# JINXER000/GIE-mapping

Hardware: AMD Instinct MI355X
Metric: edt_map_update_throughput (higher is better)
Workload: dtype int32; 1 GPU; 512x512x512 @ 0.05 m, sensor-less hash world (BASELINE config 5): occupied iff hash(x,y,z) < 1 %, full observation, 25 ~; preset=c5, fast_mode=False, tiles=single volume, blocks=360448

## Files before the change

gie-mapping_amd/csrc/gie_functors.h:

```cpp
#ifndef GIE_FUNCTORS_H
#define GIE_FUNCTORS_H

#include "gie_ops.h"


struct op_classify_depth {
    GIE_DEVM bool tile_skip(const gie_ctx &, int, int, int) const { return false; } const float *img; gie_cam_param p;
    GIE_DEVM bool skip(const gie_ctx &, int, int, int, int) const { return false; }
    GIE_DEVM void operator()(const gie_ctx &c, int x, int y, int z) const {
        const int t = gie_classify_depth(c, img, p, x, y, z);
        if (t != GIE_VOX_UNKNOWN) { c.inst_type[gie_lid(c, x, y, z)] = (int8_t)t; gie_mark_block_needed(c, x, y, z); } } };
struct op_classify_multiscan {
    const float *img; gie_multiscan_param p; float tan_lo, tan_hi; int fov_test;
    GIE_DEVM bool tile_skip(const gie_ctx &c, int x, int y, int z0) const {
        if (!fov_test || c.for_motion_planner || !(tan_hi >= 0.f && tan_lo <= 0.f)) return false;
        const float w = c.voxel_width;
        const int z1 = (z0 + 7 < c.Z) ? z0 + 7 : c.Z - 1;
        float ax, ay, az, bx, by, bz;
        gie_se3_apply(c.G2L, (float)(x + c.pvt[0]) * w, (float)(y + c.pvt[1]) * w, (float)(z0 + c.pvt[2]) * w, &ax, &ay, &az);
        gie_se3_apply(c.G2L, (float)(x + c.pvt[0]) * w, (float)(y + c.pvt[1]) * w, (float)(z1 + c.pvt[2]) * w, &bx, &by, &bz);
        const float ha = sqrtf(ay * ay + ax * ax), hb = sqrtf(by * by + bx * bx);
        return (az > ha * tan_hi && bz > hb * tan_hi) || (az < ha * tan_lo && bz < hb * tan_lo);
    }
    GIE_DEVM bool skip(const gie_ctx &c, int, int x, int y, int z) const {
// ... 40 lines not shown
    GIE_DEVM void load1(const gie_ctx &c, int id, int x, int y, int z, st &s) const { gie_mark_load1(c, id, x, y, z, s); }
    GIE_DEVM void load2(const gie_ctx &c, int, int, int, int, st &s) const { gie_mark_load2(c, s); }
    GIE_DEVM int finish(const gie_ctx &c, int id, int x, int y, int z, const st &s) const { gie_mark_finish(c, id, x, y, z, s); return 0; }
    GIE_DEVM void operator()(const gie_ctx &c, int x, int y, int z) const { gie_mark_voxel(c, x, y, z); } };
struct op_markc {
    typedef gie_markc_st st;
    GIE_DEVM bool tile_skip(const gie_ctx &c, int x, int y, int z0) const { return !c.tknown[gie_tile_index(c, x, y, z0)]; }
    GIE_DEVM bool skip(const gie_ctx &c, int id, int, int, int) const { return c.glb_type[id] == GIE_VOX_UNKNOWN; }
    GIE_DEVM void load1(const gie_ctx &c, int id, int x, int y, int z, st &s) const { gie_markc_load1(c, id, x, y, z, s); }
    GIE_DEVM void load2(const gie_ctx &c, int, int, int, int, st &s) const { gie_markc_load2(c, s); }
    GIE_DEVM int finish(const gie_ctx &c, int id, int x, int y, int z, const st &s) const { return gie_markc_finish(c, id, x, y, z, s); }
    GIE_DEVM void column_max(const gie_ctx &c, int x, int y, int z0, unsigned known, unsigned valid, int vmax) const { gie_markc_column(c, x, y, z0, known, valid, vmax); }
    GIE_DEVM int operator()(const gie_ctx &c, int x, int y, int z) const { return gie_markc_voxel(c, x, y, z); } };
struct op_commit {
    typedef gie_commit_st st;
    GIE_DEVM bool tile_skip(const gie_ctx &c, int x, int y, int z0) const { return c.cnt[GIE_CNT_BARFAIL] != 0 || !c.tknown[gie_tile_index(c, x, y, z0)]; }
    GIE_DEVM bool skip(const gie_ctx &c, int id, int, int, int) const { return c.glb_type[id] == GIE_VOX_UNKNOWN; }
    GIE_DEVM void load1(const gie_ctx &c, int id, int x, int y, int z, st &s) const { gie_commit_load1(c, id, x, y, z, s); }
    GIE_DEVM void load2(const gie_ctx &, int, int, int, int, st &) const {}
    GIE_DEVM int finish(const gie_ctx &c, int id, int, int, int, const st &s) const { gie_commit_finish(c, id, s); return 0; }
    GIE_DEVM void operator()(const gie_ctx &c, int x, int y, int z) const { gie_commit_voxel(c, x, y, z); } };

struct op_frontier {
    typedef gie_frontier_st st;
    GIE_DEVM bool tile_skip(const gie_ctx &c, int x, int y, int z0) const { return c.tsum[gie_tile_index(c, x, y, z0)] == 0; }
    GIE_DEVM bool skip(const gie_ctx &c, int id, int x, int y, int z) const {
        if (c.glb_type[id] == GIE_VOX_UNKNOWN) return true;
        const bool on_face = x == 0 || y == 0 || z == 0 || x == c.X - 1 || y == c.Y - 1 || z == c.Z - 1;
        return !on_face && c.tsum[gie_tile_index(c, x, y, z)] == 2;
    }
    GIE_DEVM void load1(const gie_ctx &c, int id, int x, int y, int z, st &s) const { gie_frontier_load1(c, id, x, y, z, s); }
    GIE_DEVM void load2(const gie_ctx &, int, int, int, int, st &) const {}
    GIE_DEVM int finish(const gie_ctx &c, int id, int x, int y, int z, const st &s) const { push_seed(c, gie_frontier_finish(c, id, x, y, z, s), id); return 0; }
    GIE_DEVM void operator()(const gie_ctx &c, int x, int y, int z) const { push_seed(c, gie_frontier_voxel(c, x, y, z), gie_lid(c, x, y, z)); }
    GIE_DEVM void push_seed(const gie_ctx &c, const int push, const int id) const {
        const unsigned long long m = __ballot(push);
        if (m) {
            const int lane = __lane_id();
            const int leader = __ffsll((long long)m) - 1;
            int base = 0;
            if (lane == leader) base = gie_aadd32(&c.cnt[GIE_CNT_C], __popcll(m));
            base = __shfl(base, leader);
            if (push) {
                const int slot = base + __popcll(m & ((1ull << lane) - 1ull));
                if (slot < c.qcap_c) c.qc[0][slot] = id;
                else gie_aor32(&c.cnt[GIE_CNT_ERR], GIE_ERRF_QUEUE);
            }
        }
    }
};

struct op_tile_summary {
    GIE_DEVM static int unk(const gie_ctx &c, int t) { return c.tunk[t] | (c.tact[t] ^ 1); }
    GIE_DEVM static uint8_t value(const gie_ctx &c, int t) {
        if (!c.tknown[t]) return 0;
        const int tx = t % c.tfd[0], ty = (t / c.tfd[0]) % c.tfd[1], tz = t / (c.tfd[0] * c.tfd[1]);
        const bool face = tx == 0 || ty == 0 || tz == 0 || tx == c.tfd[0] - 1 || ty == c.tfd[1] - 1 || tz == c.tfd[2] - 1;
        const int sx = 1, sy = c.tfd[0], sz = c.tfd[0] * c.tfd[1];
        int w = unk(c, t) | c.tflag[t];
        if (tx > 0) w |= unk(c, t - sx) | c.tflag[t - sx];
        if (tx < c.tfd[0] - 1) w |= unk(c, t + sx) | c.tflag[t + sx];
        if (ty > 0) w |= unk(c, t - sy) | c.tflag[t - sy];
        if (ty < c.tfd[1] - 1) w |= unk(c, t + sy) | c.tflag[t + sy];
        if (tz > 0) w |= unk(c, t - sz) | c.tflag[t - sz];
        if (tz < c.tfd[2] - 1) w |= unk(c, t + sz) | c.tflag[t + sz];
        return w ? 1 : (face ? 2 : 0);
    }
    GIE_DEVM void operator()(const gie_ctx &c, int t) const {
        const bool real = t >= 0;
        if (!real) t = 0;
        const uint8_t v = real ? value(c, t) : 0;
        if (real) c.tsum[t] = v;
        const int slot = gie_wg_reserve(&c.cnt[GIE_CNT_TL_FRONT], v == 1);
        if (slot >= 0) c.tl_front[slot] = t | (c.tlazy[t] ? (int32_t)0x80000000 : 0);
    } };
struct op_halo_export { int face; gie_halo_voxel *out; GIE_DEVM void operator()(const gie_ctx &c, int i) const { gie_halo_export_voxel(c, face, i, out); } };
struct op_halo_need { int face; const gie_halo_voxel *in; GIE_DEVM void operator()(const gie_ctx &c, int i) const { gie_halo_need_voxel(c, face, i, in); } };
struct op_halo_import { int face; const gie_halo_voxel *in; GIE_DEVM void operator()(const gie_ctx &c, int i) const { gie_halo_import_voxel(c, face, i, in); } };
struct op_halo_export_sparse { int face; gie_halo_entry *out; int32_t *count; GIE_DEVM void operator()(const gie_ctx &c, int i) const { gie_halo_export_sparse_voxel(c, face, i, out, count); } };
struct op_halo_need_sparse { int face, nface; const gie_halo_entry *in; const int32_t *count; GIE_DEVM void operator()(const gie_ctx &c, int j) const { gie_halo_need_entry(c, face, j, in, count, nface); } };
struct op_halo_import_sparse { int face, nface; const gie_halo_entry *in; const int32_t *count; GIE_DEVM void operator()(const gie_ctx &c, int j) const { gie_halo_import_entry(c, face, j, in, count, nface); } };
struct gie_face_set { int off[7]; GIE_DEVM int face_of(int i) const { int f = 0; while (f < 5 && i >= off[f + 1]) f++; return f; } };
struct op_halo_export_all { gie_face_set fs; gie_halo_voxel *out[6];
    GIE_DEVM void operator()(const gie_ctx &c, int i) const { const int f = fs.face_of(i); gie_halo_export_voxel(c, f, i - fs.off[f], out[f]); } };
struct op_halo_need_all { gie_face_set fs; const gie_halo_voxel *in[6];
    GIE_DEVM void operator()(const gie_ctx &c, int i) const { const int f = fs.face_of(i); gie_halo_need_voxel(c, f, i - fs.off[f], in[f]); } };
struct op_halo_import_all { gie_face_set fs; const gie_halo_voxel *in[6];
    GIE_DEVM void operator()(const gie_ctx &c, int i) const { const int f = fs.face_of(i); gie_halo_import_voxel(c, f, i - fs.off[f], in[f]); } };
struct op_refine { GIE_DEVM void operator()(const gie_ctx &c, int j) const {
        const int id = gie_refine_entry(c, j);
        if (id >= 0 && gie_refine_voxel(c, id)) gie_push32(c, c.qc[0], &c.cnt[GIE_CNT_C], c.qcap_c, id);
    } };
struct op_register_point { const float *xyz; float *g; GIE_DEVM void operator()(const gie_ctx &c, int i) const { gie_register_point(c, xyz, g, i); } };
struct op_query { const int32_t *xyz; gie_voxel *out; GIE_DEVM void operator()(const gie_ctx &c, int i) const { gie_query_voxel(c, xyz, i, out); } };
struct op_fuse_list { GIE_DEVM void operator()(const gie_ctx &c, int t) const {
        const int v = t >= 0 ? gie_fuse_tile_listed(c, t) : 0;
        const int slot = gie_wg_reserve(&c.cnt[GIE_CNT_TL_FUSE], v != 0);
        if (slot >= 0) c.tl_front[slot] = t;
    } };
struct op_pair_flush { gie_flush_boxes b; GIE_DEVM void operator()(const gie_ctx &c, int i) const { gie_pair_flush_voxel(c, b, i); } };
struct op_nbr_check { int32_t *bad; GIE_DEVM void operator()(const gie_ctx &c, int i) const {
        const int slot = i / 6, k = i - 6 * slot;
        if (slot >= c.pool_count[0] || c.g_key[slot] == GIE_KEY_EMPTY) return;
        int b[3];
        gie_unpack_crd(c.g_key[slot], &b[0], &b[1], &b[2]);
        b[k >> 1] += (k & 1) ? 1 : -1;
        const int row = c.g_nbr[8 * (size_t)slot + k];
        const int named = (row >= 0 && row < c.max_blocks && c.g_key[row] == gie_pack_crd(b[0], b[1], b[2])) ? row : -1;
        if (named != gie_hash_find(c, b[0], b[1], b[2])) {
            gie_aadd32(bad, 1);
        }
    } };
struct op_evict { GIE_DEVM void operator()(const gie_ctx &c, int slot) const { if (slot < c.pool_count[0]) gie_evict_slot(c, slot); } };
struct op_rehash { GIE_DEVM void operator()(const gie_ctx &c, int slot) const { if (slot < c.pool_count[0]) gie_rehash_slot(c, slot); } };
struct op_stream_list { const int32_t *rank; int32_t *list; GIE_DEVM void operator()(const gie_ctx &c, int i) const { gie_stream_list(c, rank, list, i); } };
struct op_stream_gather { const int32_t *list; int first; int32_t *keys; gie_voxel *out;
    GIE_DEVM void operator()(const gie_ctx &c, int i) const { gie_stream_gather(c, list, first, keys, out, i); } };
struct op_stream_clear { const int32_t *list; int first; GIE_DEVM void operator()(const gie_ctx &c, int i) const { gie_stream_clear(c, list, first, i); } };
struct op_export_pair { int32_t *d; int32_t *coc; GIE_DEVM void operator()(const gie_ctx &c, int i) const { gie_export_pair(c, i, d, coc); } };
// ... 9 lines not shown
```

gie-mapping_amd/csrc/gie_hip.hip:

```cpp
#include <cstdio>
#include <unistd.h>
#include <cstring>
#include <cstdlib>
#include <string>
#include <algorithm>
#include <vector>
#include <hip/hip_runtime.h>
#include <hip/hip_ext.h>
#include <rocprim/rocprim.hpp>
#include "gie_kernels.hip.h"

#define GIE_NEV 8

struct be_state {
    int device;
    int num_cu;
    int cu_total;
    hipStream_t stream;
    hipEvent_t ev[GIE_NEV];
    int ev_set[GIE_NEV];
    void *scan_tmp; size_t scan_bytes;
    void *arena;
    hipEvent_t copy_ev[2];
    hipStream_t side;
    hipEvent_t side_ready, side_done; int side_on, side_busy;
    int prof_on;
    std::vector<hipEvent_t> *pool;
    std::vector<int> *pending;
    int pool_used;
    int cur_id;
    double acc_ms[32]; int acc_n[32];
};

struct be_arena { char *base; size_t size, top; int k; std::vector<long long> skew; };
static void gie_set_err(const std::string &s);

#define GIE_HIP_OK(expr) do { hipError_t e_ = (expr); if (e_ != hipSuccess) { gie_set_err(std::string(#expr) + ": " + hipGetErrorString(e_)); } } while (0)

#include <mutex>
static std::mutex g_waves_mutex;
static hipEvent_t g_waves_event[64];
static bool g_waves_event_set[64];
static int g_live_mappers[64];

static int be_init(be_state *b, int device, int wave_workgroups)
{
    int n = 0;
    if (hipGetDeviceCount(&n) != hipSuccess || n <= 0) { gie_set_err("no HIP device visible (libgie_hip.so needs an AMD GPU; there is no CPU fallback)"); return 1; }
    if (device < 0 || device >= n) { gie_set_err("bad device_id"); return 1; }
    b->device = device;
    if (hipSetDevice(device) != hipSuccess) { gie_set_err("hipSetDevice failed"); return 1; }
    { hipDeviceProp_t pr; b->num_cu = (hipGetDeviceProperties(&pr, device) == hipSuccess && pr.multiProcessorCount > 0) ? pr.multiProcessorCount : 64; }
    b->cu_total = b->num_cu;
    b->num_cu = b->num_cu >= 64 ? b->num_cu / 2 : b->num_cu;
    if (wave_workgroups > 0) b->num_cu = wave_workgroups < b->cu_total ? wave_workgroups : b->cu_total;
    {
        int per_cu = 0, per_cu_c = 0;
        hipError_t oe = hipOccupancyMaxActiveBlocksPerMultiprocessor(&per_cu, reinterpret_cast<const void *>(&k_waves_ab), GIE_WAVE_THREADS, 0);
        if (oe == hipSuccess) oe = hipOccupancyMaxActiveBlocksPerMultiprocessor(&per_cu_c, reinterpret_cast<const void *>(&k_waves_c), GIE_WAVE_THREADS, 0);
        if (per_cu_c < per_cu) per_cu = per_cu_c;
        if (oe != hipSuccess || per_cu < 1) {
            gie_set_err(std::string("the wavefront kernels cannot be resident on this device (occupancy query: ") + hipGetErrorString(oe) + ", " + std::to_string(per_cu) + " workgroups per compute unit)");
            (void)hipGetLastError();
            return 1;
        }
        if (b->num_cu > per_cu * b->cu_total) b->num_cu = per_cu * b->cu_total;
    }
    if (hipStreamCreateWithFlags(&b->stream, hipStreamNonBlocking) != hipSuccess) { gie_set_err("hipStreamCreate failed"); return 1; }
    for (int i = 0; i < GIE_NEV; i++) { GIE_HIP_OK(hipEventCreate(&b->ev[i])); b->ev_set[i] = 0; }
    b->scan_tmp = nullptr; b->scan_bytes = 0; b->arena = nullptr; b->side_on = 0; b->side_busy = 0;
    for (int i = 0; i < 2; i++) GIE_HIP_OK(hipEventCreateWithFlags(&b->copy_ev[i], hipEventDisableTiming));
    b->prof_on = 0; b->cur_id = -1; b->pool = new std::vector<hipEvent_t>(); b->pending = new std::vector<int>(); b->pool_used = 0;
    for (int i = 0; i < 32; i++) { b->acc_ms[i] = 0; b->acc_n[i] = 0; }
    {
        std::lock_guard<std::mutex> lock(g_waves_mutex);
        if (++g_live_mappers[device & 63] == 2) (void)hipDeviceSynchronize();
    }
    return 0;
}
static void be_fini(be_state *b)
{
    { std::lock_guard<std::mutex> lock(g_waves_mutex); g_live_mappers[b->device & 63]--; }
    if (b->scan_tmp) (void)hipFree(b->scan_tmp);
    for (hipEvent_t e : *b->pool) (void)hipEventDestroy(e);
    delete b->pool; delete b->pending;
    for (int i = 0; i < GIE_NEV; i++) (void)hipEventDestroy(b->ev[i]);
    for (int i = 0; i < 2; i++) (void)hipEventDestroy(b->copy_ev[i]);
    (void)hipStreamDestroy(b->stream);
    if (b->side_on) { (void)hipStreamSynchronize(b->side); (void)hipEventDestroy(b->side_ready); (void)hipEventDestroy(b->side_done); (void)hipStreamDestroy(b->side); }
    if (b->arena) { be_arena *a = (be_arena *)b->arena; if (a->base) (void)hipFree(a->base); delete a; b->arena = nullptr; }
}
static be_arena *be_arena_of(be_state *b)
{
#if !defined(GIE_TEST_HOOKS)
    (void)b; return nullptr;
#else
    static const char *e = getenv("GIE_ARENA_MB");
    if (!e || atoll(e) <= 0) return nullptr;
    if (!b->arena) {
        be_arena *a = new be_arena();
        a->size = (size_t)atoll(e) << 20; a->top = 0; a->k = 0; a->base = nullptr;
        if (const char *sk = getenv("GIE_ARENA_SKEW")) { std::string t(sk); size_t i = 0; while (i < t.size()) { size_t j = t.find(',', i); if (j == std::string::npos) j = t.size(); a->skew.push_back(atoll(t.substr(i, j - i).c_str())); i = j + 1; } }
        if (hipMalloc((void **)&a->base, a->size) != hipSuccess) { a->base = nullptr; a->size = 0; }
        b->arena = a;
    }
    return (be_arena *)b->arena;
#endif
}
static void *be_alloc(be_state *b, size_t bytes, bool zero)
{
    void *p = nullptr;
    (void)hipSetDevice(b->device);
    be_arena *a = bytes >= ((size_t)64 << 20) ? be_arena_of(b) : nullptr;
    if (a && a->base) {
        const size_t sk = (size_t)((a->k < (int)a->skew.size() ? a->skew[a->k] : 0) << 20);
        const size_t at = ((a->top + ((size_t)2 << 20) - 1) & ~(((size_t)2 << 20) - 1)) + sk;
        if (at + bytes <= a->size) { p = a->base + at; a->top = at + bytes; a->k++; }
    }
    if (!p && hipMalloc(&p, bytes ? bytes : 1) != hipSuccess) return nullptr;
    if (zero) GIE_HIP_OK(hipMemsetAsync(p, 0, bytes, b->stream));
    return p;
}
static void be_free(be_state *b, void *p)
{
    (void)hipStreamSynchronize(b->stream);
    be_arena *a = (be_arena *)b->arena;
    if (a && a->base && (char *)p >= a->base && (char *)p < a->base + a->size) return;
    (void)hipFree(p);
}
static void be_memset(be_state *b, void *p, int v, size_t bytes) { GIE_HIP_OK(hipMemsetAsync(p, v, bytes, b->stream)); }
static void be_h2d(be_state *b, void *d, const void *h, size_t bytes)
{
    GIE_HIP_OK(hipMemcpyAsync(d, h, bytes, hipMemcpyHostToDevice, b->stream));
    GIE_HIP_OK(hipStreamSynchronize(b->stream));
}
static void be_d2h(be_state *b, void *h, const void *d, size_t bytes)
// ... 205 lines not shown
}
static int be_edt_z_stream(be_state *b, const gie_ctx &c, int full);
static void be_edt_z_rest(be_state *b, const gie_ctx &c, int full, int zs)
{
    if (zs == 2) gie_launch_edt_dim(b, c, c.X, false, full, 0, true);
    gie_launch_edt_dim(b, c, c.Z, true, full);
}
static void be_edt_z(be_state *b, const gie_ctx &c, int full) { be_edt_z_rest(b, c, full, be_edt_z_stream(b, c, full) ? be_zs_mode(c) : 0); }
#define GIE_VOXA_MULT 32
template <bool STAGED, class F> static void be_vox_list(be_state *b, const gie_ctx &c, const F &f, const int32_t *list, int count_idx, int always_list)
{
    GIE_LAUNCH(b, (k_voxa<F, STAGED>), dim3(b->cu_total * GIE_VOXA_MULT), dim3(256), 0, c, f, list, count_idx, always_list);
}
#define GIE_MARKC_MULT 64
#define GIE_MARKC_LAZY_MULT 40
static void be_markc(be_state *b, const gie_ctx &c, const int32_t *list)
{
    const dim3 g(b->cu_total * ((c.coc_defer && c.lazy_ok) ? GIE_MARKC_LAZY_MULT : GIE_MARKC_MULT)), t(256);
    GIE_LAUNCH(b, k_markc, g, t, 0, c, list);
}
static float be_place_probe(be_state *b, const gie_ctx &c, int reps, int streams = 15)
{
    const long long ntile = (long long)c.tfd[0] * c.tfd[1] * c.tfd[2];
    const int nslot = (int)(ntile < c.max_blocks ? ntile : c.max_blocks);
    hipEvent_t e0, e1;
    if (hipEventCreate(&e0) != hipSuccess || hipEventCreate(&e1) != hipSuccess) return -1.f;
    std::vector<float> ms;
    hipLaunchKernelGGL(k_place_probe, dim3(b->cu_total * GIE_MARKC_MULT), dim3(256), 0, b->stream, c, nslot, streams);
    for (int r = 0; r < reps; r++) {
        (void)hipEventRecord(e0, b->stream);
        hipLaunchKernelGGL(k_place_probe, dim3(b->cu_total * GIE_MARKC_MULT), dim3(256), 0, b->stream, c, nslot, streams);
        (void)hipEventRecord(e1, b->stream);
        (void)hipEventSynchronize(e1);
        float t = 0.f; (void)hipEventElapsedTime(&t, e0, e1); ms.push_back(t);
    }
    (void)hipEventDestroy(e0); (void)hipEventDestroy(e1);
    std::sort(ms.begin(), ms.end());
    GIE_HIP_OK(hipMemsetAsync(c.pair, 0, (size_t)c.N * sizeof(uint64_t), b->stream));
    return ms.empty() ? -1.f : ms[ms.size() / 2];
}
#define GIE_ROWS_MULT 32
static void be_fuse(be_state *b, const gie_ctx &c, const int32_t *list)
{
    if (c.pntcld_mode) GIE_LAUNCH(b, k_fuse_rows<true>, dim3(b->cu_total * GIE_ROWS_MULT), dim3(256), 0, c, op_fuse(), list);
    else GIE_LAUNCH(b, k_fuse_rows<false>, dim3(b->cu_total * GIE_ROWS_MULT), dim3(256), 0, c, op_fuse(), list);
}
static void be_frontier_tiles(be_state *b, const gie_ctx &c, const int32_t *known, int known_idx, const int32_t *list, int count_idx)
{
    gie_face_patches fp;
    const int da[6] = { c.Y, c.Y, c.X, c.X, c.X, c.X }, db[6] = { c.Z, c.Z, c.Z, c.Z, c.Y, c.Y };
    fp.off[0] = 0;
    for (int f = 0; f < 6; f++) { fp.na[f] = (da[f] + 7) / 8; fp.off[f + 1] = fp.off[f] + fp.na[f] * ((db[f] + 7) / 8); }
    const long long ntile = (long long)c.tfd[0] * c.tfd[1] * c.tfd[2];
    int nsum = (int)((ntile + 64 * GIE_FF_WAVES - 1) / (64 * GIE_FF_WAVES));
    if (nsum > 2 * b->cu_total) nsum = 2 * b->cu_total;
    const int nface = (fp.off[6] + GIE_FF_WAVES - 1) / GIE_FF_WAVES;
    GIE_LAUNCH(b, k_frontier_faces, dim3(nsum + nface), dim3(64 * GIE_FF_WAVES), 0, c, fp, known, known_idx, nsum);
    static int mult = 0;
    if (mult <= 0) {
        if (hipOccupancyMaxActiveBlocksPerMultiprocessor(&mult, reinterpret_cast<const void *>(&k_frontier_tiles), 64 * GIE_FR_WAVES, 0) != hipSuccess || mult < 1) mult = 2;
    }
    GIE_LAUNCH(b, k_frontier_tiles, dim3(b->cu_total * mult), dim3(64 * GIE_FR_WAVES), 0, c, list, count_idx);
}
static void be_edt_z_direct(be_state *b, const gie_ctx &c)
{
    GIE_LAUNCH(b, k_edt_z_direct, dim3(b->cu_total * 16), dim3(256), 0, c);
}
#define GIE_ZSTREAM_WAVES 8
static int be_edt_z_stream(be_state *b, const gie_ctx &c, int full)
{
    const int zs = be_zs_mode(c);
    if (!zs) return 0;
    const int nxr = (c.X + 63) / 64;
    const long long want = (long long)b->cu_total * 4 * GIE_ZSTREAM_WAVES;
    int nseg = (int)((want + (long long)nxr * c.Y - 1) / ((long long)nxr * c.Y));
    const int maxseg = c.Z / 64 > 0 ? c.Z / 64 : 1;
    if (nseg > maxseg) nseg = maxseg; if (nseg < 1) nseg = 1;
    int seg_len = ((c.Z + nseg - 1) / nseg + 31) & ~31;
    nseg = (c.Z + seg_len - 1) / seg_len;
    const long long waves = (long long)nxr * nseg * c.Y;
    long long grid = (waves + 3) / 4;
    const long long cap = (long long)b->cu_total * 8 * 4;
    if (grid > cap) grid = cap;
    if (!full && grid < (long long)b->cu_total * 16) grid = (long long)b->cu_total * 16;
    if (zs == 2) GIE_LAUNCH(b, k_edt_z_stream<true>, dim3((unsigned)grid), dim3(256), 0, c, full, nseg, seg_len, zs);
    else GIE_LAUNCH(b, k_edt_z_stream<false>, dim3((unsigned)grid), dim3(256), 0, c, full, nseg, seg_len, zs);
    return 1;
}
static void be_tile_oldskip(be_state *b, const gie_ctx &c, const int pupvt[3])
{
    const int ntile = c.tfd[0] * c.tfd[1] * c.tfd[2];
    int32_t *const count = &c.cnt[GIE_CNT_STATE1];
    GIE_LAUNCH(b, k_tile_oldskip, dim3((ntile + 255) / 256), dim3(256), 0, c, ntile, c.wc_list[0], count);
    if (c.catchup_fast) GIE_LAUNCH(b, k_coc_catchup_new, dim3(b->cu_total * 8), dim3(256), 0, c, pupvt[0], pupvt[1], pupvt[2], c.wc_list[0], count);
}
static void be_pair_materialise(be_state *b, const gie_ctx &c, int stay)
{
    const int ntile = c.tfd[0] * c.tfd[1] * c.tfd[2];
    int32_t *const count = &c.cnt[GIE_CNT_STATE2];
    GIE_LAUNCH(b, k_pair_lazy_list, dim3((ntile + 255) / 256), dim3(256), 0, c, ntile, stay, c.wc_list[1], count);
    GIE_LAUNCH(b, k_pair_lazy_run, dim3(b->cu_total * 8), dim3(256), 0, c, c.wc_list[1], count);
}
static void be_coc_catchup(be_state *b, const gie_ctx &c, const gie_catchup &p)
{
    const int ntile = c.tfd[0] * c.tfd[1] * c.tfd[2];
    int32_t *const count = &c.cnt[GIE_CNT_STATE1];
    GIE_HIP_OK(hipMemsetAsync(count, 0, sizeof(int32_t), b->stream));
    GIE_LAUNCH(b, k_coc_catchup_list, dim3((ntile + 255) / 256), dim3(256), 0, c, p, ntile, c.wc_list[0], count);
    GIE_LAUNCH(b, k_coc_catchup_run, dim3(b->cu_total * 4), dim3(256), 0, c, p, c.wc_list[0], count);
}
static void be_edt_prep(be_state *b, const gie_ctx &c)
{
    const int ncol = c.tfd[0] * c.tfd[1];
    GIE_LAUNCH(b, k_edt_prep, dim3((ncol + GIE_PREP_WAVES - 1) / GIE_PREP_WAVES), dim3(64 * GIE_PREP_WAVES), 0, c, ncol);
}
// ... 63 lines not shown
```

gie-mapping_amd/csrc/gie_kernels.hip.h:

```cpp
#ifndef GIE_KERNELS_HIP_H
#define GIE_KERNELS_HIP_H

#include <hip/hip_runtime.h>
#include "gie_functors.h"

#if defined(GIE_WAVE_TIMING) || defined(GIE_RAY_TIMING)
#include "../../tools/measure/gie_timing.h"
#endif
#if !defined(GIE_WAVE_TIMING)
#define GIE_TS2(tag, n) do { } while (0)
#define GIE_WPROF_DECL do { } while (0)
#define GIE_WPROF_MARK(base) do { } while (0)
#define GIE_WPROF_ADD(i, v) do { } while (0)
#define GIE_WPROF_END(base) do { } while (0)
#define GIE_WPROF_DRAIN() do { } while (0)
#define GIE_WPROF_SUB(i) do { } while (0)
#define GIE_WPROF_SUBSTART() do { } while (0)
#define GIE_WPROF_DUMP() do { } while (0)
#define GIE_WPROF_CLK() 0ull
#define GIE_WAVE_TIMING_RESET(cond) do { } while (0)
#endif
#if !defined(GIE_RAY_TIMING)
#define GIE_RTS(k) do { } while (0)
#endif
// ... 1647 lines not shown
        const int nz = min(8, c.Z - z0);
        int8_t ty[8]; uint32_t bc[8];
#pragma unroll
        for (int k = 0; k < 8; k++) { const size_t id = id0 + (size_t)(k < nz ? k : 0) * plane; ty[k] = (streams & 1) ? c.glb_type[id] : (int8_t)k; bc[k] = (streams & 2) ? c.bcoc[id] : (uint32_t)x; }
        const int t = gie_tile_index(c, x, y, z0);
        const gie_vaddr base = (gie_vaddr)(t % nslot) * GIE_VBSZ + ((x & 7) | ((y & 7) << 3));
#pragma unroll
        for (int k = 0; k < 8; k++) {
            if (k >= nz) break;
            const uint64_t pr = ((uint64_t)bc[k] << 20) | (uint64_t)(uint8_t)ty[k];
            if (streams & 4) c.pair[id0 + (size_t)k * plane] = pr;
            if (streams & 8) c.g_coc[base + (k << 6)] = pr ^ 0x5555ull;
            if (!(streams & 12) && pr == 0x123456789abcull) c.pair[id0] = pr;
        }
    }
}

#define GIE_FR_CQ 256
struct gie_fr_tile { uint64_t pair[512], hpair[6][64]; int32_t cq[GIE_FR_CQ]; uint8_t typ[512], htyp[6][64]; };
struct gie_nbpair_lds {
    const gie_fr_tile *L; int ex, ey, ez;
    __device__ __forceinline__ uint64_t operator()(int k, int) const {
        const int dx[6] = { -1, 1, 0, 0, 0, 0 }, dy[6] = { 0, 0, -1, 1, 0, 0 }, dz[6] = { 0, 0, 0, 0, -1, 1 };
        const int ux = ex + dx[k], uy = ey + dy[k], uz = ez + dz[k];
        const bool inside = (unsigned)ux < 8u && (unsigned)uy < 8u && (unsigned)uz < 8u;
        const int hp = (k < 2) ? (ey + 8 * ez) : ((k < 4) ? (ex + 8 * ez) : (ex + 8 * ey));
        return inside ? L->pair[ux + 8 * uy + 64 * uz] : L->hpair[k][hp];
    }
};
struct gie_absink_none { static constexpr bool outside = false; __device__ __forceinline__ void ab(const gie_ctx &, int, uint64_t, int) const {} };
__device__ __forceinline__ void gie_frontier_flush_c(const gie_ctx &c, const int32_t *cq, int &ncq, const int lane)
{
    if (ncq == 0) return;
    gie_wave_sync();
    int base = 0;
    if (lane == 0) base = atomicAdd(&c.cnt[GIE_CNT_C], ncq);
    base = __shfl(base, 0);
    for (int e = lane; e < ncq; e += 64) {
        if (base + e < c.qcap_c) c.qc[0][base + e] = cq[e];
        else atomicOr(&c.cnt[GIE_CNT_ERR], GIE_ERRF_QUEUE);
    }
    gie_wave_sync();
    ncq = 0;
}

#define GIE_FR_SRC 16u
__device__ __forceinline__ uint32_t gie_fr_srcbit(const gie_ctx &c, const uint64_t pr)
{
    int nw[3];
    gie_unpack_wr(gie_pair_par(pr), &nw[0], &nw[1], &nw[2]);
    const int n0 = nw[0] + c.upvt[0] - c.pvt[0], n1 = nw[1] + c.upvt[1] - c.pvt[1], n2 = nw[2] + c.upvt[2] - c.pvt[2];
    return (!gie_in_loc(c, n0, n1, n2) && gie_in_wr(c, nw[0], nw[1], nw[2])) ? GIE_FR_SRC : 0u;
}
__device__ __forceinline__ void gie_frontier_tile(const gie_ctx &c, gie_fr_tile &L, const int te, const int lane, int &ncq)
{
    const int t = te & 0x7fffffff;
    const int tx = t % c.tfd[0], ty = (t / c.tfd[0]) % c.tfd[1], tz = t / (c.tfd[0] * c.tfd[1]);
    const int x0 = tx * 8, y0 = ty * 8, z0 = tz * 8;
    const int lx = lane & 7, ly = lane >> 3;
    const int x = x0 + lx, y = y0 + ly;
    const bool colin = x < c.X && y < c.Y;
    const size_t plane = (size_t)c.X * c.Y;
    const size_t col = (size_t)y * c.X + x;
    uint64_t pv[8], hv[6];
    int8_t tv[8], ht[6];
    const bool lz = te < 0;
#pragma unroll
    for (int j = 0; j < 8; j++) {
        const bool in = colin && z0 + j < c.Z;
        const size_t id = in ? (size_t)(z0 + j) * plane + col : 0;
        tv[j] = c.glb_type[id];
        pv[j] = lz ? gie_pair_of_bcoc(c, c.bcoc_lazy[id], x, y, z0 + j) : c.pair[id];
        if (!in) tv[j] = -1;
    }
    {
        const int a = lane & 7, b = lane >> 3;
        const int hx[6] = { x0 - 1, x0 + 8, x0 + a, x0 + a, x0 + a, x0 + a };
        const int hy[6] = { y0 + a, y0 + a, y0 - 1, y0 + 8, y0 + b, y0 + b };
        const int hz[6] = { z0 + b, z0 + b, z0 + b, z0 + b, z0 - 1, z0 + 8 };
#pragma unroll
        for (int f = 0; f < 6; f++) {
            const bool in = gie_in_loc(c, hx[f], hy[f], hz[f]);
            const int id = in ? gie_lid(c, hx[f], hy[f], hz[f]) : 0;
            ht[f] = c.glb_type[id];
            hv[f] = gie_pair_get(c, id, in ? hx[f] : 0, in ? hy[f] : 0, in ? hz[f] : 0);
            if (!in) ht[f] = -1;
        }
    }
#pragma unroll
    for (int j = 0; j < 8; j++) {
        L.pair[lane + 64 * j] = pv[j];
        L.typ[lane + 64 * j] = tv[j] < 0 ? (uint8_t)GIE_VOX_UNKNOWN : (uint8_t)((uint32_t)(tv[j] & 15) | gie_fr_srcbit(c, pv[j]));
    }
#pragma unroll
    for (int f = 0; f < 6; f++) {
        L.hpair[f][lane] = hv[f];
        L.htyp[f][lane] = ht[f] < 0 ? (uint8_t)GIE_VOX_UNKNOWN : (uint8_t)((uint32_t)(ht[f] & 15) | gie_fr_srcbit(c, hv[f]));
    }
    gie_wave_sync();
    const unsigned long long lt = (1ull << lane) - 1ull;
    const bool xyface = x == 0 || x == c.X - 1 || y == 0 || y == c.Y - 1;
#pragma unroll 1
    for (int ez = 0; ez < 8; ez++) {
        const int vz = z0 + ez;
        const bool go = colin && vz < c.Z && !xyface && vz != 0 && vz != c.Z - 1;
        const int v = lane + 64 * ez;
        const uint32_t own = L.typ[v];
        uint32_t nn[6], src = 0;
        bool unk = false;
        const int dx[6] = { -1, 1, 0, 0, 0, 0 }, dy[6] = { 0, 0, -1, 1, 0, 0 }, dz[6] = { 0, 0, 0, 0, -1, 1 };
#pragma unroll
        for (int k = 0; k < 6; k++) {
            const int ux = lx + dx[k], uy = ly + dy[k], uz = ez + dz[k];
            const bool inside = (unsigned)ux < 8u && (unsigned)uy < 8u && (unsigned)uz < 8u;
            const int hp = (k < 2) ? (ly + 8 * ez) : ((k < 4) ? (lx + 8 * ez) : (lx + 8 * ly));
            nn[k] = inside ? L.typ[ux + 8 * uy + 64 * uz] : L.htyp[k][hp];
            src |= ((nn[k] >> 4) & 1u) << k;
            unk |= (nn[k] & 15u) == (uint32_t)GIE_VOX_UNKNOWN;
        }
        const bool need = go && (own & 15u) != (uint32_t)GIE_VOX_UNKNOWN && (src != 0u || ((own & 15u) == (uint32_t)GIE_VOX_FREE && unk));
        if (__ballot(need) == 0ull) continue;
        int push = 0, id = 0;
        if (need) {
            id = gie_lid(c, x, y, vz);
            gie_frontier_st s;
            s.p0 = L.pair[v];
            s.tys = own & 15u;
            s.tfm = src;
#pragma unroll
            for (int k = 0; k < 6; k++) s.tys |= (nn[k] & 15u) << (4 * (k + 1));
            const gie_nbpair_lds nb = { &L, lx, ly, ez };
            push = gie_frontier_finish_nb(c, id, x, y, vz, s, nb, gie_absink_none());
        }
        const unsigned long long m = __ballot(push);
        if (m) {
            if (push) L.cq[ncq + __popcll(m & lt)] = id;
            ncq += __popcll(m);
            if (ncq > GIE_FR_CQ - 64) gie_frontier_flush_c(c, L.cq, ncq, lane);
        }
    }
    gie_wave_sync();
}
#define GIE_FR_WAVES 4
__global__ __launch_bounds__(64 * GIE_FR_WAVES) void k_frontier_tiles(const gie_ctx c, const int32_t *list, const int count_idx)
{
    __shared__ gie_fr_tile s_tiles[GIE_FR_WAVES];
    const int n = c.cnt[count_idx];
    const int lane = threadIdx.x & 63, wave = threadIdx.x >> 6;
    const int stride = gridDim.x * GIE_FR_WAVES;
    int ncq = 0;
    int e = blockIdx.x * GIE_FR_WAVES + wave;
    int t = e < n ? list[e] : 0;
    while (e < n) {
        const int tn = e + stride < n ? list[e + stride] : 0;
        gie_frontier_tile(c, s_tiles[wave], t, lane, ncq);
        t = tn; e += stride;
    }
    gie_frontier_flush_c(c, s_tiles[wave].cq, ncq, lane);
}

#define GIE_FR_ABIT ((uint64_t)1 << 63)
#ifndef GIE_FF_WAVES
#define GIE_FF_WAVES 8
#endif
#define GIE_FF_AB (64 * GIE_FF_WAVES * 3)
struct gie_ff_wg { uint64_t ab_crd[GIE_FF_AB]; gie_vaddr ab_addr[GIE_FF_AB]; int32_t cq[64 * GIE_FF_WAVES]; int32_t nab, ncq, base[3], pad_; };
struct gie_absink_lds {
    static constexpr bool outside = true;
    gie_ff_wg *L;
    __device__ __forceinline__ void ab(const gie_ctx &c, int push, uint64_t crd, gie_vaddr a) const {
        if (!push) return;
        const int i = __hip_atomic_fetch_add(&L->nab, 1, __ATOMIC_RELAXED, __HIP_MEMORY_SCOPE_WORKGROUP);
        if (i < GIE_FF_AB) { L->ab_crd[i] = crd | (push == 2 ? GIE_FR_ABIT : (uint64_t)0); L->ab_addr[i] = (gie_vaddr)a; }
        else if (push == 2) gie_push64a(c, c.qa, c.qa_a, &c.cnt[GIE_CNT_A], c.qcap_ab, crd, a);
        else gie_push64a(c, c.qb, c.qb_a, &c.cnt[GIE_CNT_B], c.qcap_ab, crd, a);
    }
};
struct gie_face_patches { int off[7], na[6]; };
__global__ __launch_bounds__(64 * GIE_FF_WAVES) void k_frontier_faces(const gie_ctx c, const gie_face_patches fp, const int32_t *known, const int known_idx, const int nsum)
{
    if ((int)blockIdx.x < nsum) {
        const int n = c.cnt[known_idx];
        const op_tile_summary f;
        for (int e0 = blockIdx.x * blockDim.x; e0 < n; e0 += nsum * blockDim.x) {
            const int e = e0 + (int)threadIdx.x;
            f(c, e < n ? known[e] : -1);
        }
        return;
    }
    __shared__ gie_ff_wg W;
    const int lane = threadIdx.x & 63, wave = threadIdx.x >> 6;
    if (threadIdx.x == 0) { W.nab = 0; W.ncq = 0; }
    __syncthreads();
    const int p = ((int)blockIdx.x - nsum) * GIE_FF_WAVES + wave;
    int push = 0, id = 0;
    if (p < fp.off[6]) {
        int f = 0;
#pragma unroll
        for (int k = 1; k < 6; k++) if (p >= fp.off[k]) f = k;
        const int q = p - fp.off[f], pa = q % fp.na[f], pb = q / fp.na[f];
        const int a = pa * 8 + (lane & 7), b = pb * 8 + (lane >> 3);
        const int fix = (f & 1) ? ((f == 1) ? c.X - 1 : (f == 3) ? c.Y - 1 : c.Z - 1) : 0;
        const int vx = (f < 2) ? fix : a, vy = (f < 2) ? a : ((f < 4) ? fix : b), vz = (f < 4) ? b : fix;
        bool go = vx < c.X && vy < c.Y && vz < c.Z;
        const bool fx0 = vx == 0, fx1 = vx == c.X - 1, fy0 = vy == 0, fy1 = vy == c.Y - 1, fz0 = vz == 0;
        if ((f >= 1 && fx0) || (f >= 2 && fx1) || (f >= 3 && fy0) || (f >= 4 && fy1) || (f >= 5 && fz0)) go = false;
        if (go && op_tile_summary::value(c, gie_tile_index(c, vx, vy, vz)) == 0) go = false;
        if (go) {
            id = gie_lid(c, vx, vy, vz);
            const int ox = vx + ((f == 0) ? -1 : (f == 1) ? 1 : 0), oy = vy + ((f == 2) ? -1 : (f == 3) ? 1 : 0), oz = vz + ((f == 4) ? -1 : (f == 5) ? 1 : 0);
            gie_out_pre pre;
            pre.k = f;
            pre.a = gie_gvox_tab(c, ox + c.pvt[0], oy + c.pvt[1], oz + c.pvt[2]);
            gie_frontier_st s;
            gie_frontier_load1<true>(c, id, vx, vy, vz, s);
            pre.nty = pre.a >= 0 ? c.g_type[pre.a] : (int8_t)0;
            pre.ncoc = pre.a >= 0 ? c.g_coc[pre.a] : (uint64_t)0;
            const gie_nbpair_plane nb = { c.pair };
            const gie_absink_lds sink = { &W };
            push = gie_frontier_finish_nb(c, id, vx, vy, vz, s, nb, sink, &pre);
        }
    }
    if (push) W.cq[__hip_atomic_fetch_add(&W.ncq, 1, __ATOMIC_RELAXED, __HIP_MEMORY_SCOPE_WORKGROUP)] = id;
    __syncthreads();
    const int nab = min(W.nab, GIE_FF_AB), ncq = W.ncq;
    if (nab == 0 && ncq == 0) return;
    const unsigned long long lt = (1ull << lane) - 1ull;
    if (wave == 0) {
        int na = 0;
        for (int e0 = 0; e0 < nab; e0 += 64) na += __popcll(__ballot(e0 + lane < nab && (W.ab_crd[e0 + lane] & GIE_FR_ABIT) != 0));
        if (lane < 3) {
            const int cnt = (lane == 0) ? na : (lane == 1) ? nab - na : ncq;
            int32_t *const ctr = &c.cnt[(lane == 0) ? GIE_CNT_A : (lane == 1) ? GIE_CNT_B : GIE_CNT_C];
            W.base[lane] = cnt > 0 ? gie_aadd32(ctr, cnt) : 0;
        }
        gie_wave_sync();
        int ra = W.base[0], rb = W.base[1];
        for (int e0 = 0; e0 < nab; e0 += 64) {
            const int e = e0 + lane;
            const bool have = e < nab;
            const uint64_t crd = have ? W.ab_crd[e] : (uint64_t)0;
            const bool isa = have && (crd & GIE_FR_ABIT) != 0, isb = have && !isa;
// ... 1343 lines not shown
```

Baseline: 101,200 Mvoxels/s.

## Precompute per-tile halo masks in summary pass to skip clean neighbor loads

The tile-summary pass now scans all tiles in a dense grid instead of the known-tile list. For each frontier tile it writes a 16-bit mask recording which of the six neighbouring tiles are unknown or flagged, and which of them are lazy. The frontier-tile kernel reads this mask and loads halo voxel type and pair data only from marked neighbours, choosing the lazy or direct pair path without evaluating it per voxel. This is meant to cut global memory traffic for halo voxels next to clean tiles, at the cost of a new device buffer, a dense scan over every tile, and an added __syncthreads in the tile loop.

```diff
diff --git a/gie-mapping_amd/csrc/gie_functors.h b/gie-mapping_amd/csrc/gie_functors.h
--- a/gie-mapping_amd/csrc/gie_functors.h
+++ b/gie-mapping_amd/csrc/gie_functors.h
@@ -116,19 +116,23 @@
 
 struct op_tile_summary {
     GIE_DEVM static int unk(const gie_ctx &c, int t) { return c.tunk[t] | (c.tact[t] ^ 1); }
+    GIE_DEVM static int around(const gie_ctx &c, int t) {
+        const int tx = t % c.tfd[0], ty = (t / c.tfd[0]) % c.tfd[1], tz = t / (c.tfd[0] * c.tfd[1]);
+        const int sx = 1, sy = c.tfd[0], sz = c.tfd[0] * c.tfd[1];
+        int m = (unk(c, t) | c.tflag[t]) ? 64 : 0;
+        if (tx > 0 && (unk(c, t - sx) | c.tflag[t - sx])) m |= 1;
+        if (tx < c.tfd[0] - 1 && (unk(c, t + sx) | c.tflag[t + sx])) m |= 2;
+        if (ty > 0 && (unk(c, t - sy) | c.tflag[t - sy])) m |= 4;
+        if (ty < c.tfd[1] - 1 && (unk(c, t + sy) | c.tflag[t + sy])) m |= 8;
+        if (tz > 0 && (unk(c, t - sz) | c.tflag[t - sz])) m |= 16;
+        if (tz < c.tfd[2] - 1 && (unk(c, t + sz) | c.tflag[t + sz])) m |= 32;
+        return m;
+    }
     GIE_DEVM static uint8_t value(const gie_ctx &c, int t) {
         if (!c.tknown[t]) return 0;
         const int tx = t % c.tfd[0], ty = (t / c.tfd[0]) % c.tfd[1], tz = t / (c.tfd[0] * c.tfd[1]);
         const bool face = tx == 0 || ty == 0 || tz == 0 || tx == c.tfd[0] - 1 || ty == c.tfd[1] - 1 || tz == c.tfd[2] - 1;
-        const int sx = 1, sy = c.tfd[0], sz = c.tfd[0] * c.tfd[1];
-        int w = unk(c, t) | c.tflag[t];
-        if (tx > 0) w |= unk(c, t - sx) | c.tflag[t - sx];
-        if (tx < c.tfd[0] - 1) w |= unk(c, t + sx) | c.tflag[t + sx];
-        if (ty > 0) w |= unk(c, t - sy) | c.tflag[t - sy];
-        if (ty < c.tfd[1] - 1) w |= unk(c, t + sy) | c.tflag[t + sy];
-        if (tz > 0) w |= unk(c, t - sz) | c.tflag[t - sz];
-        if (tz < c.tfd[2] - 1) w |= unk(c, t + sz) | c.tflag[t + sz];
-        return w ? 1 : (face ? 2 : 0);
+        return around(c, t) ? 1 : (face ? 2 : 0);
     }
     GIE_DEVM void operator()(const gie_ctx &c, int t) const {
         const bool real = t >= 0;
diff --git a/gie-mapping_amd/csrc/gie_hip.hip b/gie-mapping_amd/csrc/gie_hip.hip
--- a/gie-mapping_amd/csrc/gie_hip.hip
+++ b/gie-mapping_amd/csrc/gie_hip.hip
@@ -20,6 +20,7 @@
     hipEvent_t ev[GIE_NEV];
     int ev_set[GIE_NEV];
     void *scan_tmp; size_t scan_bytes;
+    uint16_t *fr_halo; long long fr_halo_n;
     void *arena;
     hipEvent_t copy_ev[2];
     hipStream_t side;
@@ -68,7 +69,7 @@
     }
     if (hipStreamCreateWithFlags(&b->stream, hipStreamNonBlocking) != hipSuccess) { gie_set_err("hipStreamCreate failed"); return 1; }
     for (int i = 0; i < GIE_NEV; i++) { GIE_HIP_OK(hipEventCreate(&b->ev[i])); b->ev_set[i] = 0; }
-    b->scan_tmp = nullptr; b->scan_bytes = 0; b->arena = nullptr; b->side_on = 0; b->side_busy = 0;
+    b->scan_tmp = nullptr; b->scan_bytes = 0; b->fr_halo = nullptr; b->fr_halo_n = 0; b->arena = nullptr; b->side_on = 0; b->side_busy = 0;
     for (int i = 0; i < 2; i++) GIE_HIP_OK(hipEventCreateWithFlags(&b->copy_ev[i], hipEventDisableTiming));
     b->prof_on = 0; b->cur_id = -1; b->pool = new std::vector<hipEvent_t>(); b->pending = new std::vector<int>(); b->pool_used = 0;
     for (int i = 0; i < 32; i++) { b->acc_ms[i] = 0; b->acc_n[i] = 0; }
@@ -82,6 +83,7 @@
 {
     { std::lock_guard<std::mutex> lock(g_waves_mutex); g_live_mappers[b->device & 63]--; }
     if (b->scan_tmp) (void)hipFree(b->scan_tmp);
+    if (b->fr_halo) (void)hipFree(b->fr_halo);
     for (hipEvent_t e : *b->pool) (void)hipEventDestroy(e);
     delete b->pool; delete b->pending;
     for (int i = 0; i < GIE_NEV; i++) (void)hipEventDestroy(b->ev[i]);
@@ -393,15 +395,23 @@
     fp.off[0] = 0;
     for (int f = 0; f < 6; f++) { fp.na[f] = (da[f] + 7) / 8; fp.off[f + 1] = fp.off[f] + fp.na[f] * ((db[f] + 7) / 8); }
     const long long ntile = (long long)c.tfd[0] * c.tfd[1] * c.tfd[2];
-    int nsum = (int)((ntile + 64 * GIE_FF_WAVES - 1) / (64 * GIE_FF_WAVES));
+    (void)known; (void)known_idx;
+    const long long nst = (long long)((c.tfd[0] + 7) / 8) * c.tfd[1] * c.tfd[2] * 8;
+    int nsum = (int)((nst + 64 * GIE_FF_WAVES - 1) / (64 * GIE_FF_WAVES));
     if (nsum > 2 * b->cu_total) nsum = 2 * b->cu_total;
     const int nface = (fp.off[6] + GIE_FF_WAVES - 1) / GIE_FF_WAVES;
-    GIE_LAUNCH(b, k_frontier_faces, dim3(nsum + nface), dim3(64 * GIE_FF_WAVES), 0, c, fp, known, known_idx, nsum);
+    if (b->fr_halo_n < ntile) {
+        if (b->fr_halo) { (void)hipStreamSynchronize(b->stream); (void)hipFree(b->fr_halo); b->fr_halo = nullptr; b->fr_halo_n = 0; }
+        GIE_HIP_OK(hipMalloc((void **)&b->fr_halo, (size_t)ntile * sizeof(uint16_t)));
+        if (!b->fr_halo) return;
+        b->fr_halo_n = ntile;
+    }
+    GIE_LAUNCH(b, k_frontier_faces, dim3(nsum + nface), dim3(64 * GIE_FF_WAVES), 0, c, fp, const_cast<int32_t *>(list), b->fr_halo, count_idx, nsum);
     static int mult = 0;
     if (mult <= 0) {
         if (hipOccupancyMaxActiveBlocksPerMultiprocessor(&mult, reinterpret_cast<const void *>(&k_frontier_tiles), 64 * GIE_FR_WAVES, 0) != hipSuccess || mult < 1) mult = 2;
     }
-    GIE_LAUNCH(b, k_frontier_tiles, dim3(b->cu_total * mult), dim3(64 * GIE_FR_WAVES), 0, c, list, count_idx);
+    GIE_LAUNCH(b, k_frontier_tiles, dim3(b->cu_total * mult), dim3(64 * GIE_FR_WAVES), 0, c, list, (const uint16_t *)b->fr_halo, count_idx);
 }
 static void be_edt_z_direct(be_state *b, const gie_ctx &c)
 {
diff --git a/gie-mapping_amd/csrc/gie_kernels.hip.h b/gie-mapping_amd/csrc/gie_kernels.hip.h
--- a/gie-mapping_amd/csrc/gie_kernels.hip.h
+++ b/gie-mapping_amd/csrc/gie_kernels.hip.h
@@ -1723,7 +1723,7 @@
     const int n0 = nw[0] + c.upvt[0] - c.pvt[0], n1 = nw[1] + c.upvt[1] - c.pvt[1], n2 = nw[2] + c.upvt[2] - c.pvt[2];
     return (!gie_in_loc(c, n0, n1, n2) && gie_in_wr(c, nw[0], nw[1], nw[2])) ? GIE_FR_SRC : 0u;
 }
-__device__ __forceinline__ void gie_frontier_tile(const gie_ctx &c, gie_fr_tile &L, const int te, const int lane, int &ncq)
+__device__ __forceinline__ void gie_frontier_tile(const gie_ctx &c, gie_fr_tile &L, const int te, const int hw, const int lane, int &ncq)
 {
     const int t = te & 0x7fffffff;
     const int tx = t % c.tfd[0], ty = (t / c.tfd[0]) % c.tfd[1], tz = t / (c.tfd[0] * c.tfd[1]);
@@ -1736,6 +1736,9 @@
     uint64_t pv[8], hv[6];
     int8_t tv[8], ht[6];
     const bool lz = te < 0;
+    bool hload[6], hlz[6];
+#pragma unroll
+    for (int f = 0; f < 6; f++) { hload[f] = (hw >> f) & 1; hlz[f] = (hw >> (8 + f)) & 1; }
 #pragma unroll
     for (int j = 0; j < 8; j++) {
         const bool in = colin && z0 + j < c.Z;
@@ -1752,9 +1755,12 @@
 #pragma unroll
         for (int f = 0; f < 6; f++) {
             const bool in = gie_in_loc(c, hx[f], hy[f], hz[f]);
-            const int id = in ? gie_lid(c, hx[f], hy[f], hz[f]) : 0;
-            ht[f] = c.glb_type[id];
-            hv[f] = gie_pair_get(c, id, in ? hx[f] : 0, in ? hy[f] : 0, in ? hz[f] : 0);
+            ht[f] = (int8_t)GIE_VOX_FREE; hv[f] = 0;
+            if (hload[f]) {
+                const int id = in ? gie_lid(c, hx[f], hy[f], hz[f]) : 0;
+                ht[f] = c.glb_type[id];
+                hv[f] = hlz[f] ? gie_pair_of_bcoc(c, c.bcoc_lazy[id], in ? hx[f] : 0, in ? hy[f] : 0, in ? hz[f] : 0) : c.pair[id];
+            }
             if (!in) ht[f] = -1;
         }
     }
@@ -1766,7 +1772,7 @@
 #pragma unroll
     for (int f = 0; f < 6; f++) {
         L.hpair[f][lane] = hv[f];
-        L.htyp[f][lane] = ht[f] < 0 ? (uint8_t)GIE_VOX_UNKNOWN : (uint8_t)((uint32_t)(ht[f] & 15) | gie_fr_srcbit(c, hv[f]));
+        L.htyp[f][lane] = ht[f] < 0 ? (uint8_t)GIE_VOX_UNKNOWN : (uint8_t)((uint32_t)(ht[f] & 15) | (hload[f] ? gie_fr_srcbit(c, hv[f]) : 0u));
     }
     gie_wave_sync();
     const unsigned long long lt = (1ull << lane) - 1ull;
@@ -1813,7 +1819,7 @@
     gie_wave_sync();
 }
 #define GIE_FR_WAVES 4
-__global__ __launch_bounds__(64 * GIE_FR_WAVES) void k_frontier_tiles(const gie_ctx c, const int32_t *list, const int count_idx)
+__global__ __launch_bounds__(64 * GIE_FR_WAVES) void k_frontier_tiles(const gie_ctx c, const int32_t *list, const uint16_t *halo, const int count_idx)
 {
     __shared__ gie_fr_tile s_tiles[GIE_FR_WAVES];
     const int n = c.cnt[count_idx];
@@ -1821,13 +1827,38 @@
     const int stride = gridDim.x * GIE_FR_WAVES;
     int ncq = 0;
     int e = blockIdx.x * GIE_FR_WAVES + wave;
-    int t = e < n ? list[e] : 0;
-    while (e < n) {
-        const int tn = e + stride < n ? list[e + stride] : 0;
-        gie_frontier_tile(c, s_tiles[wave], t, lane, ncq);
-        t = tn; e += stride;
+    int t = e < n ? list[e] : 0, hw = e < n ? halo[e] : 0;
+    for (int e0 = blockIdx.x * GIE_FR_WAVES; e0 < n; e0 += stride) {
+        const bool more = e + stride < n;
+        const int tn = more ? list[e + stride] : 0, hn = more ? halo[e + stride] : 0;
+        __syncthreads();
+        if (e < n) gie_frontier_tile(c, s_tiles[wave], t, __builtin_amdgcn_readfirstlane(hw), lane, ncq);
+        t = tn; hw = hn; e += stride;
     }
     gie_frontier_flush_c(c, s_tiles[wave].cq, ncq, lane);
+}
+
+__device__ __forceinline__ void gie_frontier_summary(const gie_ctx &c, int32_t *list, uint16_t *halo, const int count_idx, const int first, const int nwg)
+{
+    const int ngx = (c.tfd[0] + 7) >> 3;
+    const long long nthr = (long long)ngx * c.tfd[1] * c.tfd[2] * 8;
+    const int ts[3] = { 1, c.tfd[0], c.tfd[0] * c.tfd[1] };
+    for (long long i0 = (long long)first * blockDim.x; i0 < nthr; i0 += (long long)nwg * blockDim.x) {
+        const long long i = i0 + threadIdx.x;
+        const int g = (int)(i >> 3), tx = (g % ngx) * 8 + (int)(i & 7);
+        const bool real = i < nthr && tx < c.tfd[0];
+        const int t = real ? (g / ngx) * c.tfd[0] + tx : 0;
+        const uint8_t v = real ? op_tile_summary::value(c, t) : 0;
+        if (real) c.tsum[t] = v;
+        const int slot = gie_wg_reserve(&c.cnt[count_idx], v == 1);
+        if (slot >= 0) {
+            int hw = op_tile_summary::around(c, t) & 63;
+#pragma unroll
+            for (int f = 0; f < 6; f++) if (((hw >> f) & 1) && c.tlazy[t + ((f & 1) ? ts[f >> 1] : -ts[f >> 1])]) hw |= 256 << f;
+            list[slot] = t | (c.tlazy[t] ? (int32_t)0x80000000 : 0);
+            halo[slot] = (uint16_t)hw;
+        }
+    }
 }
 
 #define GIE_FR_ABIT ((uint64_t)1 << 63)
@@ -1848,17 +1879,9 @@
     }
 };
 struct gie_face_patches { int off[7], na[6]; };
-__global__ __launch_bounds__(64 * GIE_FF_WAVES) void k_frontier_faces(const gie_ctx c, const gie_face_patches fp, const int32_t *known, const int known_idx, const int nsum)
-{
-    if ((int)blockIdx.x < nsum) {
-        const int n = c.cnt[known_idx];
-        const op_tile_summary f;
-        for (int e0 = blockIdx.x * blockDim.x; e0 < n; e0 += nsum * blockDim.x) {
-            const int e = e0 + (int)threadIdx.x;
-            f(c, e < n ? known[e] : -1);
-        }
-        return;
-    }
+__global__ __launch_bounds__(64 * GIE_FF_WAVES) void k_frontier_faces(const gie_ctx c, const gie_face_patches fp, int32_t *list, uint16_t *halo, const int count_idx, const int nsum)
+{
+    if ((int)blockIdx.x < nsum) { gie_frontier_summary(c, list, halo, count_idx, blockIdx.x, nsum); return; }
     __shared__ gie_ff_wg W;
     const int lane = threadIdx.x & 63, wave = threadIdx.x >> 6;
     if (threadIdx.x == 0) { W.nab = 0; W.ncq = 0; }
```

After: 102,000 Mvoxels/s, median of 6. No clear change (+0.8%).
